# archinetai/audio-diffusion-pytorch

Hardware: AMD Instinct MI355X
Metric: denoising steps/s (UNetV0 fwd+bwd) at [B,2,2**18] (higher is better)
Workload: dtype f32; 1 GPU; BASELINE.json configs[1]: unconditional DiffusionModel(UNetV0 channels=[8,32,64,128,256,512,512,1024,1024], factors=[1,4,4,4,2,2,2,2,2], items=[1,2,2,2,2,2,2,4,4]) fwd+bwd, audio=randn(4,2,2**18) per GPU, random-init weights; per_gpu_batch=4, global_batch=4, length=262144, launch=hipGraph replay, parallelism=single, collective_world_size=1, collectives_in_graph=False, optimizer=none (the metric is fwd+bwd; gradients for all 176M parameters are produced)

## Files before the change

audio_diffusion_pytorch_amd/csrc/norm.hip:

```cpp
#include <stdlib.h>
#include "adp_rt.h"
#include "adp.h"

namespace {

constexpr int GN_CHUNK = 4096;

__global__ __launch_bounds__(256) void gn_partial_kernel(const float* x, int64_t NG, int64_t nchunks, float* ws) {
  __shared__ float sh[4];
  const int64_t bg = blockIdx.y, c = blockIdx.x;
  const float* base = x + bg * NG + c * GN_CHUNK;
  const int64_t cnt = (NG - c * GN_CHUNK) < GN_CHUNK ? (NG - c * GN_CHUNK) : GN_CHUNK;
  float v[16];
  float s = 0.0f;
#pragma unroll
  for (int j = 0; j < 16; ++j) {
    const int64_t i = (int64_t)j * 256 + threadIdx.x;
    v[j] = (i < cnt) ? base[i] : 0.0f;
    s += v[j];
  }
  const float mean = adp_block_sum<4>(s, sh) / (float)cnt;
  float q = 0.0f;
#pragma unroll
  for (int j = 0; j < 16; ++j) {
// ... 870 lines not shown
    f32x4 o;
#pragma unroll
    for (int k = 0; k < 4; ++k) o[k] = rstd[k] * (g[i][k] - m1[k] - xh[i][k] * m2[k]);
    if (dres) {
      const f32x4 r = *reinterpret_cast<const f32x4*>(dres + boff + (int64_t)c * L);
#pragma unroll
      for (int k = 0; k < 4; ++k) o[k] += r[k];
    }
    *reinterpret_cast<f32x4*>(dx + boff + (int64_t)c * L) = o;
  }
}

template <int LPR, int NT, int VPT>
__global__ __launch_bounds__(NT) void chan_lnv_bwd_chain_kernel(const float* x, const float* ss, int64_t bstride,
                                                                const float* stats1, const float* dxn, const float* gamma,
                                                                const float* stats2, const float* dres, int C, int L,
                                                                int NTL, float* dx, float* ws1, float* ws2) {
  constexpr int TL = 4 * LPR, RPP = NT / LPR, NW = NT / 64;
  __shared__ float red[4][NW][TL];
  const int tid = threadIdx.x, lane = tid & 63, wave = tid >> 6;
  const int lr = tid % LPR, rg = tid / LPR;
  const int tile = blockIdx.x, l0 = tile * TL + 4 * lr, b = blockIdx.y;
  const bool valid = l0 < L;
  const int64_t boff = (int64_t)b * C * L + l0;
  float mean1[4] = {0.0f, 0.0f, 0.0f, 0.0f}, rstd1[4] = {0.0f, 0.0f, 0.0f, 0.0f};
  float mean2[4] = {0.0f, 0.0f, 0.0f, 0.0f}, rstd2[4] = {0.0f, 0.0f, 0.0f, 0.0f};
  if (valid) {
    const float* sp = stats1 + ((int64_t)b * L + l0) * 2;
    const f32x4 a = *reinterpret_cast<const f32x4*>(sp), c4 = *reinterpret_cast<const f32x4*>(sp + 4);
    mean1[0] = a[0], rstd1[0] = a[1], mean1[1] = a[2], rstd1[1] = a[3];
    mean1[2] = c4[0], rstd1[2] = c4[1], mean1[3] = c4[2], rstd1[3] = c4[3];
    const float* sq = stats2 + ((int64_t)b * L + l0) * 2;
    const f32x4 e = *reinterpret_cast<const f32x4*>(sq), f4 = *reinterpret_cast<const f32x4*>(sq + 4);
    mean2[0] = e[0], rstd2[0] = e[1], mean2[1] = e[2], rstd2[1] = e[3];
    mean2[2] = f4[0], rstd2[2] = f4[1], mean2[3] = f4[2], rstd2[3] = f4[3];
  }
  const float* sb = ss + b * bstride;
  f32x4 xh[VPT], g[VPT];
  float mulv[VPT], addv[VPT];
  float s1[4] = {0.0f, 0.0f, 0.0f, 0.0f}, s2[4] = {0.0f, 0.0f, 0.0f, 0.0f};
  auto xhat2 = [&](int i, int k) {
    return (fmaf(xh[i][k], mulv[i], addv[i]) - mean2[k]) * rstd2[k];
  };
#pragma unroll
  for (int i = 0; i < VPT; ++i) {
    const int c = rg + i * RPP;
    const bool ok = valid && c < C;
    f32x4 d;
    if (ok) {
      d = *reinterpret_cast<const f32x4*>(dxn + boff + (int64_t)c * L);
      xh[i] = *reinterpret_cast<const f32x4*>(x + boff + (int64_t)c * L);
    } else {
#pragma unroll
      for (int k = 0; k < 4; ++k) d[k] = xh[i][k] = 0.0f;
    }
    mulv[i] = (c < C) ? 1.0f + sb[c] : 0.0f;
    addv[i] = (c < C) ? sb[C + c] : 0.0f;
    const float gm = (c < C) ? gamma[c] : 0.0f;
    float pa = 0.0f, pb = 0.0f;
#pragma unroll
    for (int k = 0; k < 4; ++k) {
      xh[i][k] = ok ? (xh[i][k] - mean1[k]) * rstd1[k] : 0.0f;
      const float x2 = ok ? xhat2(i, k) : 0.0f;
      g[i][k] = d[k] * gm;
      s1[k] += g[i][k];
      s2[k] = fmaf(g[i][k], x2, s2[k]);
      pa = fmaf(d[k], x2, pa);
      pb += d[k];
    }
#pragma unroll
    for (int o = 1; o < LPR; o <<= 1) {
      pa += __shfl_xor(pa, o, 64);
      pb += __shfl_xor(pb, o, 64);
    }
    if (lr == 0 && c < C) {
      ws2[(((int64_t)b * 2 + 0) * NTL + tile) * C + c] = pa;
      ws2[(((int64_t)b * 2 + 1) * NTL + tile) * C + c] = pb;
    }
  }
  auto over_channels = [&](float (&a)[4], float (&c2)[4], int stage) {
#pragma unroll
    for (int o = LPR; o < 64; o <<= 1)
#pragma unroll
      for (int k = 0; k < 4; ++k) {
        a[k] += __shfl_xor(a[k], o, 64);
        c2[k] += __shfl_xor(c2[k], o, 64);
      }
    if (NW > 1) {
      if (lane < LPR)
#pragma unroll
        for (int k = 0; k < 4; ++k) {
          red[2 * stage][wave][4 * lr + k] = a[k];
          red[2 * stage + 1][wave][4 * lr + k] = c2[k];
        }
      __syncthreads();
#pragma unroll
      for (int k = 0; k < 4; ++k) {
        float u = 0.0f, w2 = 0.0f;
#pragma unroll
        for (int w = 0; w < NW; ++w) {
          u += red[2 * stage][w][4 * lr + k];
          w2 += red[2 * stage + 1][w][4 * lr + k];
        }
        a[k] = u, c2[k] = w2;
      }
    }
#pragma unroll
    for (int k = 0; k < 4; ++k) {
      a[k] /= (float)C;
      c2[k] /= (float)C;
    }
  };
  over_channels(s1, s2, 0);
  float t1[4] = {0.0f, 0.0f, 0.0f, 0.0f}, t2[4] = {0.0f, 0.0f, 0.0f, 0.0f};
#pragma unroll
  for (int i = 0; i < VPT; ++i) {
    const int c = rg + i * RPP;
    const bool ok = valid && c < C;
    f32x4 r = f32x4{0.0f, 0.0f, 0.0f, 0.0f};
    if (ok && dres) r = *reinterpret_cast<const f32x4*>(dres + boff + (int64_t)c * L);
    float pa = 0.0f, pb = 0.0f;
#pragma unroll
    for (int k = 0; k < 4; ++k) {
      const float o = ok ? rstd2[k] * (g[i][k] - s1[k] - xhat2(i, k) * s2[k]) + r[k] : 0.0f;
      pa = fmaf(o, xh[i][k], pa);
      pb += o;
      g[i][k] = o * mulv[i];
      t1[k] += g[i][k];
      t2[k] = fmaf(g[i][k], xh[i][k], t2[k]);
    }
#pragma unroll
    for (int o = 1; o < LPR; o <<= 1) {
      pa += __shfl_xor(pa, o, 64);
      pb += __shfl_xor(pb, o, 64);
    }
    if (lr == 0 && c < C) {
      ws1[(((int64_t)b * 2 + 0) * NTL + tile) * C + c] = pa;
      ws1[(((int64_t)b * 2 + 1) * NTL + tile) * C + c] = pb;
    }
  }
  over_channels(t1, t2, 1);
  if (!valid) return;
#pragma unroll
  for (int i = 0; i < VPT; ++i) {
    const int c = rg + i * RPP;
    if (c >= C) continue;
    f32x4 o;
#pragma unroll
    for (int k = 0; k < 4; ++k) o[k] = rstd1[k] * (g[i][k] - t1[k] - xh[i][k] * t2[k]);
    *reinterpret_cast<f32x4*>(dx + boff + (int64_t)c * L) = o;
  }
}

struct LnvCfg {
  int lpr, nt, vpt;
};
static LnvCfg lnv_cfg(int64_t C, int64_t B, int64_t L, bool bwd = false) {
  if (C <= 8) return {64, 256, 2};
  if (C <= 32) return {32, 256, 4};
  if (C <= 64) return {16, 256, 4};
  if (C <= 128) return {8, 256, 4};
  if (C <= 256) {
    if (adp_knob(bwd ? "ADP_LNV_NT_BWD" : "ADP_LNV_NT", 512) == 1024) return {8, 1024, 2};
    return {8, 512, 4};
  }
  int lpr = 4;
  while (lpr > 1 && B * adp_cdiv(L, 4 * lpr) < 32) lpr >>= 1;
  if (adp_knob(bwd ? "ADP_LNV_NT_BWD" : "ADP_LNV_NT", 512) != 1024) {
    const int lp = (C <= 512 && lpr == 1) ? 2 : lpr;
    return {lp, 512, C <= 512 ? lp : 2 * lp};
  }
  if (C <= 512) return {lpr == 1 ? 2 : lpr, 1024, lpr == 4 ? 2 : 1};
  return {lpr, 1024, lpr};
}
static bool lnv_ok(int64_t L, const void* a, const void* b, const void* c, const void* d, const void* e) {
  return (L & 3) == 0 && ((reinterpret_cast<uintptr_t>(a) | reinterpret_cast<uintptr_t>(b) | reinterpret_cast<uintptr_t>(c) |
                           reinterpret_cast<uintptr_t>(d) | reinterpret_cast<uintptr_t>(e)) & 15) == 0;
}

struct LnCfg {
  int tl, nt;
};
LnCfg ln_cfg(int64_t C, int64_t B, int64_t L) {
  if (C <= 64) return {64, 256};
  if (C <= 128) return {32, 256};
  if (C <= 256) return {32, 1024};
  if (B * adp_cdiv(L, 16) >= 192) return {16, 1024};
  if (B * adp_cdiv(L, 8) >= 192) return {8, 1024};
  return {4, 1024};
}
constexpr int64_t LN_CMAX = 1024;

int launch_ln_fwd(const float* x, const float* ss, int64_t bstride, int64_t B, int64_t C, int64_t L, float eps, float* y,
                  float* stats, void* stream, const float* gam = nullptr, const float* bet = nullptr,
                  const float* gam2 = nullptr, const float* bet2 = nullptr, float* y2 = nullptr, float eps2 = 0.0f,
                  float* cy = nullptr, float* cstats = nullptr) {
  if (cy && !(lnv_ok(L, x, y, y2, stats, cy) && lnv_ok(L, cstats, nullptr, nullptr, nullptr, nullptr))) {
    const int rc = launch_ln_fwd(x, ss, bstride, B, C, L, eps, y, stats, stream);
    if (rc != ADP_OK) return rc;
    return launch_ln_fwd(y, nullptr, 0, B, C, L, eps2, cy, cstats, stream, gam, bet, gam2, bet2, y2);
  }
  if (lnv_ok(L, x, y, y2, stats, nullptr)) {
    const LnvCfg v = lnv_cfg(C, B, L);
    dim3 vgrid((unsigned)adp_cdiv(L, 4 * v.lpr), (unsigned)B);
#define ADP_LNV_FWD(LPR, NT, VPT)                                                                                     \
  if (v.lpr == LPR && v.nt == NT && v.vpt == VPT) {                                                                   \
    ADP_LAUNCH((chan_lnv_fwd_kernel<LPR, NT, VPT>), vgrid, dim3(NT), stream, x, ss, bstride, (int)C, (int)L, eps, y, \
               stats, gam, bet, gam2, bet2, y2, eps2, cy, cstats);                                                    \
    return ADP_LAUNCH_OK();                                                                                           \
  }
    ADP_LNV_FWD(64, 256, 2) ADP_LNV_FWD(32, 256, 4) ADP_LNV_FWD(16, 256, 4) ADP_LNV_FWD(8, 256, 4) ADP_LNV_FWD(8, 1024, 2)
    ADP_LNV_FWD(4, 1024, 2) ADP_LNV_FWD(2, 1024, 1) ADP_LNV_FWD(4, 1024, 4) ADP_LNV_FWD(2, 1024, 2) ADP_LNV_FWD(1, 1024, 1)
    ADP_LNV_FWD(4, 512, 4) ADP_LNV_FWD(4, 512, 8) ADP_LNV_FWD(2, 512, 2) ADP_LNV_FWD(2, 512, 4) ADP_LNV_FWD(1, 512, 2) ADP_LNV_FWD(8, 512, 4)
#undef ADP_LNV_FWD
  }
  const LnCfg k = ln_cfg(C, B, L);
  dim3 grid((unsigned)adp_cdiv(L, k.tl), (unsigned)B);
  if (k.tl == 8)
    ADP_LAUNCH((chan_ln_fwd_kernel<8, 1024, 8>), grid, dim3(1024), stream, x, ss, bstride, (int)C, (int)L, eps, y, stats, gam, bet, gam2, bet2, y2);
  else if (k.tl == 4)
    ADP_LAUNCH((chan_ln_fwd_kernel<4, 1024, 4>), grid, dim3(1024), stream, x, ss, bstride, (int)C, (int)L, eps, y, stats, gam, bet, gam2, bet2, y2);
  else if (k.tl == 64 && C <= 8)
    ADP_LAUNCH((chan_ln_fwd_kernel<64, 256, 2>), grid, dim3(256), stream, x, ss, bstride, (int)C, (int)L, eps, y, stats, gam, bet, gam2, bet2, y2);
  else if (k.tl == 64 && C <= 32)
    ADP_LAUNCH((chan_ln_fwd_kernel<64, 256, 8>), grid, dim3(256), stream, x, ss, bstride, (int)C, (int)L, eps, y, stats, gam, bet, gam2, bet2, y2);
  else if (k.tl == 64)
    ADP_LAUNCH((chan_ln_fwd_kernel<64, 256, 16>), grid, dim3(256), stream, x, ss, bstride, (int)C, (int)L, eps, y, stats, gam, bet, gam2, bet2, y2);
  else if (k.tl == 32 && k.nt == 256)
    ADP_LAUNCH((chan_ln_fwd_kernel<32, 256, 16>), grid, dim3(256), stream, x, ss, bstride, (int)C, (int)L, eps, y, stats, gam, bet, gam2, bet2, y2);
  else if (k.tl == 32)
    ADP_LAUNCH((chan_ln_fwd_kernel<32, 1024, 8>), grid, dim3(1024), stream, x, ss, bstride, (int)C, (int)L, eps, y, stats, gam, bet, gam2, bet2, y2);
  else
    ADP_LAUNCH((chan_ln_fwd_kernel<16, 1024, 16>), grid, dim3(1024), stream, x, ss, bstride, (int)C, (int)L, eps, y, stats, gam, bet, gam2, bet2, y2);
  return ADP_LAUNCH_OK();
}

int launch_ln_bwd(const float* x, const float* dy, const float* ss, int64_t bstride, const float* gamma,
                  const float* stats, const float* dres, int64_t B, int64_t C, int64_t L, float* dx, float* ws,
                  void* stream) {
  if (lnv_ok(L, x, dy, dres, dx, stats)) {
    const LnvCfg v = lnv_cfg(C, B, L, true);
    const int VNTL = (int)adp_cdiv(L, 4 * v.lpr);
    dim3 vgrid((unsigned)VNTL, (unsigned)B);
#define ADP_LNV_BWD(LPR, NT, VPT)                                                                                      \
  if (v.lpr == LPR && v.nt == NT && v.vpt == VPT) {                                                                    \
    ADP_LAUNCH((chan_lnv_bwd_kernel<LPR, NT, VPT>), vgrid, dim3(NT), stream, x, dy, ss, bstride, gamma, stats, dres,  \
               (int)C, (int)L, VNTL, dx, ws);                                                                          \
    return VNTL;                                                                                                       \
  }
    ADP_LNV_BWD(64, 256, 2) ADP_LNV_BWD(32, 256, 4) ADP_LNV_BWD(16, 256, 4) ADP_LNV_BWD(8, 256, 4) ADP_LNV_BWD(8, 1024, 2)
    ADP_LNV_BWD(4, 1024, 2) ADP_LNV_BWD(2, 1024, 1) ADP_LNV_BWD(4, 1024, 4) ADP_LNV_BWD(2, 1024, 2) ADP_LNV_BWD(1, 1024, 1)
    ADP_LNV_BWD(4, 512, 4) ADP_LNV_BWD(4, 512, 8) ADP_LNV_BWD(2, 512, 2) ADP_LNV_BWD(2, 512, 4) ADP_LNV_BWD(1, 512, 2) ADP_LNV_BWD(8, 512, 4)
#undef ADP_LNV_BWD
  }
  const LnCfg k = ln_cfg(C, B, L);
  const int NTL = (int)adp_cdiv(L, k.tl);
  dim3 grid((unsigned)NTL, (unsigned)B);
  if (k.tl == 8)
    ADP_LAUNCH((chan_ln_bwd_kernel<8, 1024, 8>), grid, dim3(1024), stream, x, dy, ss, bstride, gamma, stats, dres,
               (int)C, (int)L, NTL, dx, ws);
  else if (k.tl == 4)
    ADP_LAUNCH((chan_ln_bwd_kernel<4, 1024, 4>), grid, dim3(1024), stream, x, dy, ss, bstride, gamma, stats, dres,
               (int)C, (int)L, NTL, dx, ws);
  else if (k.tl == 64 && C <= 8)
    ADP_LAUNCH((chan_ln_bwd_kernel<64, 256, 2>), grid, dim3(256), stream, x, dy, ss, bstride, gamma, stats, dres,
               (int)C, (int)L, NTL, dx, ws);
  else if (k.tl == 64 && C <= 32)
    ADP_LAUNCH((chan_ln_bwd_kernel<64, 256, 8>), grid, dim3(256), stream, x, dy, ss, bstride, gamma, stats, dres,
               (int)C, (int)L, NTL, dx, ws);
  else if (k.tl == 64)
    ADP_LAUNCH((chan_ln_bwd_kernel<64, 256, 16>), grid, dim3(256), stream, x, dy, ss, bstride, gamma, stats, dres,
               (int)C, (int)L, NTL, dx, ws);
  else if (k.tl == 32 && k.nt == 256)
    ADP_LAUNCH((chan_ln_bwd_kernel<32, 256, 16>), grid, dim3(256), stream, x, dy, ss, bstride, gamma, stats, dres,
               (int)C, (int)L, NTL, dx, ws);
  else if (k.tl == 32)
    ADP_LAUNCH((chan_ln_bwd_kernel<32, 1024, 8>), grid, dim3(1024), stream, x, dy, ss, bstride, gamma, stats, dres,
               (int)C, (int)L, NTL, dx, ws);
  else
    ADP_LAUNCH((chan_ln_bwd_kernel<16, 1024, 16>), grid, dim3(1024), stream, x, dy, ss, bstride, gamma, stats, dres,
               (int)C, (int)L, NTL, dx, ws);
  return NTL;
}

__global__ __launch_bounds__(256) void reduce_rows_kernel(const float* ws, int64_t B, int64_t W, int64_t NT,
                                                          int64_t bstride, int sum_over_b, int accumulate,
                                                          float* out) {
  const int lane = threadIdx.x & 63, wave = threadIdx.x >> 6;
  const int64_t row = (int64_t)blockIdx.x * 4 + wave;
  const int64_t rows = sum_over_b ? W : B * W;
  if (row >= rows) return;
  float s = 0.0f;
  if (sum_over_b) {
    for (int64_t b = 0; b < B; ++b)
      for (int64_t t = lane; t < NT; t += 64) s += ws[(b * W + row) * NT + t];
  } else {
    for (int64_t t = lane; t < NT; t += 64) s += ws[row * NT + t];
  }
  s = adp_wave_sum(s);
  if (lane == 0) {
    const int64_t o = sum_over_b ? row : (row / W) * bstride + (row % W);
    out[o] = accumulate ? out[o] + s : s;
  }
}

__global__ __launch_bounds__(1024) void reduce_tiles_kernel(const float* ws, int64_t B, int64_t C, int64_t NT,
                                                            int64_t bstride, int sum_over_b, int accumulate,
                                                            float* out) {
  __shared__ float part[16][64];
  const int lane = threadIdx.x & 63, tg = threadIdx.x >> 6;
  const int64_t W = 2 * C;
  const int64_t j = (int64_t)blockIdx.x * 64 + lane;
  const int64_t bb = blockIdx.y;
  float s = 0.0f;
  if (j < W) {
    const int64_t which = j / C, c = j % C;
    const int64_t b0 = sum_over_b ? 0 : bb, b1 = sum_over_b ? B : bb + 1;
    for (int64_t b = b0; b < b1; ++b) {
      const float* p = ws + ((b * 2 + which) * NT) * C + c;
      for (int64_t t = tg; t < NT; t += 16) s += p[t * C];
    }
  }
  part[tg][lane] = s;
  __syncthreads();
  if (tg == 0 && j < W) {
    float v = 0.0f;
#pragma unroll
    for (int k = 0; k < 16; ++k) v += part[k][lane];
    const int64_t o = sum_over_b ? j : bb * bstride + j;
    out[o] = accumulate ? out[o] + v : v;
  }
}

__global__ __launch_bounds__(256) void reduce_tiles_wave_kernel(const float* ws, int64_t B, int64_t C, int64_t NT,
                                                                int64_t bstride, int sum_over_b, int accumulate,
                                                                float* out) {
  const int lane = threadIdx.x & 63, wave = threadIdx.x >> 6;
  const int64_t i = (int64_t)blockIdx.x * 4 + wave;
  const int64_t W = 2 * C;
  const int64_t total = sum_over_b ? W : B * W;
  if (i >= total) return;
  const int64_t j = i % W, which = j / C, c = j % C;
  float s = 0.0f;
  const int64_t b0 = sum_over_b ? 0 : i / W, b1 = sum_over_b ? B : b0 + 1;
  for (int64_t b = b0; b < b1; ++b) {
    const float* p = ws + ((b * 2 + which) * NT) * C + c;
    for (int64_t t = lane; t < NT; t += 64) s += p[t * C];
  }
  s = adp_wave_sum(s);
  if (lane == 0) {
    const int64_t o = sum_over_b ? j : b0 * bstride + j;
    out[o] = accumulate ? out[o] + s : s;
  }
}

static void launch_reduce_tiles(const float* ws, int64_t B, int64_t C, int64_t NT, int64_t bstride, int sum_over_b,
                                int accumulate, float* out, void* stream) {
  const int64_t total = sum_over_b ? 2 * C : B * 2 * C;
  if (NT >= 128 && C <= 64)
    ADP_LAUNCH(reduce_tiles_wave_kernel, dim3((unsigned)adp_cdiv(total, 4)), dim3(256), stream, ws, B, C, NT, bstride,
               sum_over_b, accumulate, out);
  else
    ADP_LAUNCH(reduce_tiles_kernel, dim3((unsigned)adp_cdiv(2 * C, 64), (unsigned)(sum_over_b ? 1 : B)), dim3(1024),
               stream, ws, B, C, NT, bstride, sum_over_b, accumulate, out);
}

constexpr int MOD_BATCH = 8;
struct adp_mod_batch {
  const float* ws[MOD_BATCH];
  float* out[MOD_BATCH];
};

__global__ __launch_bounds__(1024) void reduce_tiles_batch_kernel(adp_mod_batch q, int64_t C, int64_t NT, int64_t bstride) {
  __shared__ float part[16][64];
  const int lane = threadIdx.x & 63, tg = threadIdx.x >> 6;
  const int64_t W = 2 * C;
  const int64_t j = (int64_t)blockIdx.x * 64 + lane;
  const int64_t b = blockIdx.y;
  const float* ws = q.ws[blockIdx.z];
  float s = 0.0f;
  if (j < W) {
    const int64_t which = j / C, c = j % C;
    const float* p = ws + ((b * 2 + which) * NT) * C + c;
    for (int64_t t = tg; t < NT; t += 16) s += p[t * C];
  }
  part[tg][lane] = s;
  __syncthreads();
  if (tg == 0 && j < W) {
    float v = 0.0f;
#pragma unroll
    for (int k = 0; k < 16; ++k) v += part[k][lane];
    q.out[blockIdx.z][b * bstride + j] = v;
// ... 86 lines not shown
  if (B <= 0 || C <= 0 || L <= 0 || G <= 0 || C % G) return ADP_ERR_SHAPE;
  const int64_t NG = (C / G) * L, nchunks = adp_cdiv(NG, GN_CHUNK);
  if (B * G > 65535 || B * C > 65535) return ADP_ERR_SHAPE;
  ADP_LAUNCH(gn_partial_kernel, dim3((unsigned)nchunks, (unsigned)(B * G)), dim3(256), stream, x, NG, nchunks, ws);
  if ((L & 3) == 0 && ((reinterpret_cast<uintptr_t>(x) | reinterpret_cast<uintptr_t>(act)) & 15) == 0)
    return launch_gn_act_slab<2>(x, ws, gamma, beta, B, C, L, G, nchunks, eps, stats, act, stream);
  ADP_LAUNCH(gn_apply_kernel, dim3((unsigned)adp_cdiv(L, 1024), (unsigned)(B * C)), dim3(256), stream, x,
             (const float*)ws, gamma, beta, C, L, G, nchunks, eps, stats, act);
  return ADP_LAUNCH_OK();
}

extern "C" int64_t adp_row_nsplit(int64_t rows, int64_t L) { return row_nsplit(rows, L); }

extern "C" int adp_gn_silu_bwd_reduce(const float* x, const float* dact, const float* stats, const float* gamma,
                                      const float* beta, int64_t B, int64_t C, int64_t L, int64_t G, int64_t NS,
                                      float* ab, void* stream) {
  if (!x || !dact || !stats || !gamma || !beta || !ab) return ADP_ERR_NULL;
  if (B <= 0 || C <= 0 || L <= 0 || G <= 0 || C % G || NS < 1 || NS > 65535 || B * C > 65535) return ADP_ERR_SHAPE;
  int64_t CL = adp_cdiv(L, NS);
  if ((L & 3) == 0) CL = (CL + 3) & ~(int64_t)3;
  if (gn_bwd_vec_ok(x, dact, nullptr, nullptr, L, CL) && (reinterpret_cast<uintptr_t>(ab) & 7) == 0) {
    const int64_t nseg = B * C * NS;
    const int tpr = gn_bwd_tpr(CL);
    const dim3 grid((unsigned)adp_cdiv(nseg, 256 / tpr));
#define ADP_GN_RED(T) \
  ADP_LAUNCH((gn_bwd_reduce_vec_kernel<T>), grid, dim3(256), stream, x, dact, stats, gamma, beta, C, L, G, NS, CL, nseg, ab)
    if (tpr == 16) ADP_GN_RED(16);
    else if (tpr == 32) ADP_GN_RED(32);
    else if (tpr == 64) ADP_GN_RED(64);
    else ADP_GN_RED(256);
#undef ADP_GN_RED
    return ADP_LAUNCH_OK();
  }
  ADP_LAUNCH(gn_bwd_reduce_kernel, dim3((unsigned)NS, (unsigned)(B * C)), dim3(256), stream, x, dact, stats, gamma,
             beta, C, L, G, NS, CL, ab);
  return ADP_LAUNCH_OK();
}

extern "C" int adp_gn_silu_bwd_apply_ab(const float* x, const float* dact, const float* stats, const float* gamma,
                                        const float* beta, const float* ab, const float* dres, int64_t B, int64_t C,
                                        int64_t L, int64_t G, int64_t NS, int64_t NSab, float* dx, float* dgamma,
                                        float* dbeta, int64_t accumulate, void* stream) {
  if (!x || !dact || !stats || !gamma || !beta || !ab || !dx || (!dgamma != !dbeta)) return ADP_ERR_NULL;
  if (B <= 0 || C <= 0 || L <= 0 || G <= 0 || C % G || NS < 1 || NS > 65535 || NSab < 1 || B * C > 65535) return ADP_ERR_SHAPE;
  int64_t CL = adp_cdiv(L, NS);
  if ((L & 3) == 0) CL = (CL + 3) & ~(int64_t)3;
  if (gn_bwd_vec_ok(x, dact, dres, dx, L, CL) && (reinterpret_cast<uintptr_t>(ab) & 7) == 0) {
    const int64_t nseg = B * C * NS;
    const int tpr = gn_bwd_tpr(CL);
    const dim3 grid((unsigned)adp_cdiv(nseg, 256 / tpr));
#define ADP_GN_APP(T)                                                                                                  \
  ADP_LAUNCH((gn_bwd_apply_vec_kernel<T>), grid, dim3(256), stream, x, dact, stats, gamma, beta, ab, dres, C, L, G, NS, \
             CL, nseg, dx, B, dgamma, dbeta, (int)accumulate, NSab)
    if (tpr == 16) ADP_GN_APP(16);
    else if (tpr == 32) ADP_GN_APP(32);
    else if (tpr == 64) ADP_GN_APP(64);
    else ADP_GN_APP(256);
#undef ADP_GN_APP
    return ADP_LAUNCH_OK();
  }
  ADP_LAUNCH(gn_bwd_apply_kernel, dim3((unsigned)NS, (unsigned)(B * C)), dim3(256), stream, x, dact, stats, gamma,
             beta, ab, dres, C, L, G, NS, CL, dx, B, dgamma, dbeta, (int)accumulate, NSab);
  return ADP_LAUNCH_OK();
}

extern "C" int adp_gn_silu_bwd_apply(const float* x, const float* dact, const float* stats, const float* gamma,
                                     const float* beta, const float* ab, const float* dres, int64_t B, int64_t C,
                                     int64_t L, int64_t G, int64_t NS, float* dx, float* dgamma, float* dbeta,
                                     int64_t accumulate, void* stream) {
  return adp_gn_silu_bwd_apply_ab(x, dact, stats, gamma, beta, ab, dres, B, C, L, G, NS, NS, dx, dgamma, dbeta, accumulate,
                                  stream);
}

extern "C" int adp_gn_param_grad(const float* ab, int64_t B, int64_t C, int64_t NS, float* dgamma, float* dbeta,
                                 int64_t accumulate, void* stream) {
  if (!ab || !dgamma || !dbeta) return ADP_ERR_NULL;
  if (B <= 0 || C <= 0 || NS < 1) return ADP_ERR_SHAPE;
  ADP_LAUNCH(gn_param_grad_kernel, dim3((unsigned)adp_cdiv(C, 256)), dim3(256), stream, ab, B, C, NS, dgamma, dbeta,
             (int)accumulate);
  return ADP_LAUNCH_OK();
}

extern "C" int adp_modulation_fwd(const float* x, const float* ss, int64_t ss_bstride, int64_t B, int64_t C,
                                  int64_t L, float eps, float* y, float* stats, void* stream) {
  if (!x || !ss || !y || !stats) return ADP_ERR_NULL;
  if (B <= 0 || C <= 0 || L <= 0 || B > 65535 || L >= (int64_t)1 << 31) return ADP_ERR_SHAPE;
  if (C > LN_CMAX) return ADP_ERR_UNSUPPORTED;
  return launch_ln_fwd(x, ss, ss_bstride, B, C, L, eps, y, stats, stream);
}

extern "C" int adp_modulation_ln_fwd(const float* x, const float* ss, int64_t ss_bstride, int64_t B, int64_t C, int64_t L,
                                     float eps, float* y, float* stats, float eps_ln, const float* gamma, const float* beta,
                                     float* xn, const float* gamma2, const float* beta2, float* xn2, float* ln_stats,
                                     void* stream) {
  if (!x || !ss || !y || !stats || !gamma || !beta || !xn || !ln_stats) return ADP_ERR_NULL;
  if (xn2 && (!gamma2 || !beta2)) return ADP_ERR_NULL;
  if (B <= 0 || C <= 0 || L <= 0 || B > 65535 || L >= (int64_t)1 << 31) return ADP_ERR_SHAPE;
  if (C > LN_CMAX) return ADP_ERR_UNSUPPORTED;
  return launch_ln_fwd(x, ss, ss_bstride, B, C, L, eps, y, stats, stream, gamma, beta, gamma2, beta2, xn2, eps_ln, xn,
                       ln_stats);
}

extern "C" int adp_gn_finalize(const float* part, int64_t B, int64_t C, int64_t E, int64_t G, float eps, float* stats,
                               void* stream) {
  if (!part || !stats) return ADP_ERR_NULL;
  if (B <= 0 || C <= 0 || E <= 0 || G <= 0 || C % G || (C / G) % 4) return ADP_ERR_SHAPE;
  ADP_LAUNCH(gn_finalize_kernel, dim3((unsigned)(B * G)), dim3(64), stream, part, C, E, G, eps, stats);
  return ADP_LAUNCH_OK();
}

extern "C" int adp_gn_finalize_act(const float* x, const float* part, int64_t B, int64_t C, int64_t L, int64_t E,
                                   int64_t G, float eps, const float* gamma, const float* beta, float* stats,
                                   float* act, void* stream) {
  if (!x || !part || !gamma || !beta || !stats || !act) return ADP_ERR_NULL;
  if (B <= 0 || C <= 0 || L <= 0 || E <= 0 || G <= 0 || C % G || (C / G) % 4 || B * C > 65535) return ADP_ERR_SHAPE;
  if ((L & 3) == 0 && ((reinterpret_cast<uintptr_t>(x) | reinterpret_cast<uintptr_t>(act)) & 15) == 0)
    return launch_gn_act_slab<1>(x, part, gamma, beta, B, C, L, G, E, eps, stats, act, stream);
  ADP_LAUNCH(gn_finalize_act_kernel, dim3((unsigned)adp_cdiv(L, 1024), (unsigned)(B * C)), dim3(256), stream, x, part,
             gamma, beta, C, L, G, E, eps, stats, act);
  return ADP_LAUNCH_OK();
}

extern "C" int adp_gn_act(const float* x, const float* stats, const float* gamma, const float* beta, int64_t B,
                          int64_t C, int64_t L, int64_t G, float* act, void* stream) {
  if (!x || !stats || !gamma || !beta || !act) return ADP_ERR_NULL;
  if (B <= 0 || C <= 0 || L <= 0 || G <= 0 || C % G || B * C > 65535) return ADP_ERR_SHAPE;
  if ((L & 3) == 0 && ((reinterpret_cast<uintptr_t>(x) | reinterpret_cast<uintptr_t>(act)) & 15) == 0)
    return launch_gn_act_slab<0>(x, stats, gamma, beta, B, C, L, G, 0, 0.0f, (float*)nullptr, act, stream);
  ADP_LAUNCH(gn_act_kernel, dim3((unsigned)adp_cdiv(L, 1024), (unsigned)(B * C)), dim3(256), stream, x, stats, gamma,
             beta, C, L, G, act);
  return ADP_LAUNCH_OK();
}

extern "C" int adp_ln_stats(const float* x, int64_t B, int64_t C, int64_t L, float eps, float* stats, void* stream) {
  if (!x || !stats) return ADP_ERR_NULL;
  if (B <= 0 || C <= 0 || L <= 0 || B > 65535 || L >= (int64_t)1 << 31) return ADP_ERR_SHAPE;
  if (C > LN_CMAX) return ADP_ERR_UNSUPPORTED;
  return launch_ln_fwd(x, (const float*)nullptr, (int64_t)0, B, C, L, eps, (float*)nullptr, stats, stream);
}

extern "C" int adp_ln_affine_fwd(const float* x, int64_t B, int64_t C, int64_t L, float eps, const float* gamma,
                                 const float* beta, float* y, const float* gamma2, const float* beta2, float* y2,
                                 float* stats, void* stream) {
  if (!x || !gamma || !beta || !y || !stats) return ADP_ERR_NULL;
  if (y2 && (!gamma2 || !beta2)) return ADP_ERR_NULL;
  if (B <= 0 || C <= 0 || L <= 0 || B > 65535 || L >= (int64_t)1 << 31) return ADP_ERR_SHAPE;
  if (C > LN_CMAX) return ADP_ERR_UNSUPPORTED;
  return launch_ln_fwd(x, (const float*)nullptr, (int64_t)0, B, C, L, eps, y, stats, stream, gamma, beta, gamma2, beta2,
                       y2);
}

extern "C" int64_t adp_chan_ln_bwd_ws_bytes(int64_t B, int64_t C, int64_t L) {
  if (B <= 0 || C <= 0 || L <= 0) return ADP_ERR_SHAPE;
  const int64_t t_old = adp_cdiv(L, ln_cfg(C, B, L).tl), t_vec = adp_cdiv(L, 4 * lnv_cfg(C, B, L).lpr);
  return B * 2 * C * (t_old > t_vec ? t_old : t_vec) * (int64_t)sizeof(float);
}

extern "C" int adp_modulation_bwd(const float* x, const float* dy, const float* ss, int64_t ss_bstride,
                                  const float* stats, int64_t B, int64_t C, int64_t L, float* dx, float* dss,
                                  int64_t dss_bstride, float* ws, void* stream) {
  if (!x || !dy || !ss || !stats || !dx || !dss || !ws) return ADP_ERR_NULL;
  if (B <= 0 || C <= 0 || L <= 0 || B > 65535 || L >= (int64_t)1 << 31) return ADP_ERR_SHAPE;
  if (C > LN_CMAX) return ADP_ERR_UNSUPPORTED;
  const int64_t NT = launch_ln_bwd(x, dy, ss, ss_bstride, (const float*)nullptr, stats, (const float*)nullptr, B, C, L, dx,
                                   ws, stream);
  launch_reduce_tiles((const float*)ws, B, C, NT, dss_bstride, 0, 0, dss, stream);
  return ADP_LAUNCH_OK();
}

extern "C" int64_t adp_modulation_bwd_partial(const float* x, const float* dy, const float* ss, int64_t ss_bstride,
                                              const float* stats, int64_t B, int64_t C, int64_t L, float* dx, float* ws,
                                              void* stream) {
  if (!x || !dy || !ss || !stats || !dx || !ws) return ADP_ERR_NULL;
  if (B <= 0 || C <= 0 || L <= 0 || B > 65535 || L >= (int64_t)1 << 31) return ADP_ERR_SHAPE;
  if (C > LN_CMAX) return ADP_ERR_UNSUPPORTED;
  const int64_t NT = launch_ln_bwd(x, dy, ss, ss_bstride, (const float*)nullptr, stats, (const float*)nullptr, B, C, L, dx,
                                   ws, stream);
  return ADP_LAUNCH_OK() == ADP_OK ? NT : (int64_t)ADP_ERR_LAUNCH;
}

extern "C" int adp_modulation_bwd_reduce(const float* const* ws, float* const* dss, int64_t n, int64_t B, int64_t C,
                                         int64_t NT, int64_t dss_bstride, void* stream) {
  if (!ws || !dss) return ADP_ERR_NULL;
  if (n < 1 || B <= 0 || C <= 0 || NT <= 0 || B > 65535) return ADP_ERR_SHAPE;
  for (int64_t at = 0; at < n; at += MOD_BATCH) {
    adp_mod_batch q;
    const int m = (int)(n - at < MOD_BATCH ? n - at : MOD_BATCH);
    for (int i = 0; i < MOD_BATCH; ++i) {
      q.ws[i] = ws[at + (i < m ? i : 0)];
      q.out[i] = dss[at + (i < m ? i : 0)];
      if (!q.ws[i] || !q.out[i]) return ADP_ERR_NULL;
    }
    if (NT >= 128 && C <= 64)
      ADP_LAUNCH(reduce_tiles_wave_batch_kernel, dim3((unsigned)adp_cdiv(B * 2 * C, 4), 1, (unsigned)m), dim3(256), stream, q,
                 B, C, NT, dss_bstride);
    else
      ADP_LAUNCH(reduce_tiles_batch_kernel, dim3((unsigned)adp_cdiv(2 * C, 64), (unsigned)B, (unsigned)m), dim3(1024),
                 stream, q, C, NT, dss_bstride);
  }
  return ADP_LAUNCH_OK();
}

extern "C" int adp_ln_bwd(const float* x, const float* dxn, const float* stats, const float* gamma, const float* dres,
                          int64_t B, int64_t C, int64_t L, int64_t accumulate, float* dx, float* dgamma_dbeta,
                          float* ws, void* stream) {
  if (!x || !dxn || !stats || !gamma || !dx || !dgamma_dbeta || !ws) return ADP_ERR_NULL;
  if (B <= 0 || C <= 0 || L <= 0 || B > 65535 || L >= (int64_t)1 << 31) return ADP_ERR_SHAPE;
  if (C > LN_CMAX) return ADP_ERR_UNSUPPORTED;
  const int64_t NT = launch_ln_bwd(x, dxn, (const float*)nullptr, (int64_t)0, gamma, stats, dres, B, C, L, dx, ws, stream);
  launch_reduce_tiles((const float*)ws, B, C, NT, (int64_t)0, 1, (int)accumulate, dgamma_dbeta, stream);
  return ADP_LAUNCH_OK();
}

extern "C" int64_t adp_modulation_ln_bwd_partial(const float* x, const float* ss, int64_t ss_bstride, const float* stats,
                                                 const float* y, const float* dxn, const float* gamma, const float* ln_stats,
                                                 const float* dres, int64_t B, int64_t C, int64_t L, int64_t accumulate,
                                                 float* dx, float* ws, float* dgamma_dbeta, float* ws_ln, void* stream) {
  if (!x || !ss || !stats || !y || !dxn || !gamma || !ln_stats || !dx || !ws || !dgamma_dbeta || !ws_ln) return ADP_ERR_NULL;
  if (B <= 0 || C <= 0 || L <= 0 || B > 65535 || L >= (int64_t)1 << 31) return ADP_ERR_SHAPE;
  if (C > LN_CMAX) return ADP_ERR_UNSUPPORTED;
  int64_t NT = -1;
  if (lnv_ok(L, x, dxn, dres, dx, stats) && lnv_ok(L, ln_stats, nullptr, nullptr, nullptr, nullptr)) {
    const LnvCfg v = lnv_cfg(C, B, L, true);
    const int VNTL = (int)adp_cdiv(L, 4 * v.lpr);
    dim3 vgrid((unsigned)VNTL, (unsigned)B);
#define ADP_LNV_CHAIN(LPR, NT_, VPT)                                                                                    \
  if (NT < 0 && v.lpr == LPR && v.nt == NT_ && v.vpt == VPT) {                                                          \
    ADP_LAUNCH((chan_lnv_bwd_chain_kernel<LPR, NT_, VPT>), vgrid, dim3(NT_), stream, x, ss, ss_bstride, stats, dxn,    \
               gamma, ln_stats, dres, (int)C, (int)L, VNTL, dx, ws, ws_ln);                                             \
    NT = VNTL;                                                                                                          \
  }
    ADP_LNV_CHAIN(64, 256, 2) ADP_LNV_CHAIN(32, 256, 4) ADP_LNV_CHAIN(16, 256, 4) ADP_LNV_CHAIN(8, 256, 4) ADP_LNV_CHAIN(8, 1024, 2)
    ADP_LNV_CHAIN(4, 1024, 2) ADP_LNV_CHAIN(2, 1024, 1) ADP_LNV_CHAIN(4, 1024, 4) ADP_LNV_CHAIN(2, 1024, 2) ADP_LNV_CHAIN(1, 1024, 1)
    ADP_LNV_CHAIN(4, 512, 4) ADP_LNV_CHAIN(4, 512, 8) ADP_LNV_CHAIN(2, 512, 2) ADP_LNV_CHAIN(2, 512, 4) ADP_LNV_CHAIN(1, 512, 2) ADP_LNV_CHAIN(8, 512, 4)
#undef ADP_LNV_CHAIN
    if (NT > 0) launch_reduce_tiles((const float*)ws_ln, B, C, NT, (int64_t)0, 1, (int)accumulate, dgamma_dbeta, stream);
  }
  if (NT < 0) {
    const int64_t NA = launch_ln_bwd(y, dxn, (const float*)nullptr, (int64_t)0, gamma, ln_stats, dres, B, C, L, dx, ws_ln, stream);
    launch_reduce_tiles((const float*)ws_ln, B, C, NA, (int64_t)0, 1, (int)accumulate, dgamma_dbeta, stream);
    NT = launch_ln_bwd(x, dx, ss, ss_bstride, (const float*)nullptr, stats, (const float*)nullptr, B, C, L, dx, ws, stream);
  }
  return ADP_LAUNCH_OK() == ADP_OK ? NT : (int64_t)ADP_ERR_LAUNCH;
}

extern "C" int64_t adp_skipmod_bwd_ws_bytes(int64_t B, int64_t C, int64_t L) {
  if (B <= 0 || C <= 0 || L <= 0) return ADP_ERR_SHAPE;
  return B * C * row_nsplit(B * C, L) * (int64_t)sizeof(float);
}

extern "C" int adp_skipmod_bwd(const float* g, const float* x, const float* scale, int64_t scale_bstride, int64_t B,
                               int64_t C, int64_t L, float* dx, float* dscale, int64_t dscale_bstride, float* ws,
                               void* stream) {
  if (!g || !x || !scale || !dx || !dscale || !ws) return ADP_ERR_NULL;
  if (B <= 0 || C <= 0 || L <= 0 || B * C > 65535) return ADP_ERR_SHAPE;
  const int64_t NS = row_nsplit(B * C, L), CL = adp_cdiv(L, NS);
  ADP_LAUNCH(skipmod_bwd_kernel, dim3((unsigned)NS, (unsigned)(B * C)), dim3(256), stream, g, x, scale,
             scale_bstride, C, L, NS, CL, dx, ws);
  ADP_LAUNCH(reduce_rows_kernel, dim3((unsigned)adp_cdiv(B * C, 4)), dim3(256), stream, (const float*)ws, B, C, NS,
             dscale_bstride, 0, 0, dscale);
  return ADP_LAUNCH_OK();
}
```

Measured before the change: 91.27 denoising steps/s.

## Split channel LayerNorm across channel groups for low-occupancy deep layers

Adds a channel-split path for channel LayerNorm forward and backward when C is 512-1024 and there are few length tiles. Each call becomes two kernels over a 3D grid with a channel-split dimension. The first writes partial sums, using a pivoted shifted-variance scheme in forward, into scratch space (the output buffer in forward, extra workspace in backward). The second combines the partials Chan-style and applies the normalization. This spreads work across more CUs for the small-L, wide-channel levels, at the cost of an extra launch and re-reading the input.

```diff
diff --git a/audio_diffusion_pytorch_amd/csrc/norm.hip b/audio_diffusion_pytorch_amd/csrc/norm.hip
--- a/audio_diffusion_pytorch_amd/csrc/norm.hip
+++ b/audio_diffusion_pytorch_amd/csrc/norm.hip
@@ -1046,6 +1046,308 @@
   }
 }
 
+struct LnsCfg {
+  int vpt, cs;
+};
+static LnsCfg lns_cfg(int64_t C, int64_t B, int64_t L) {
+  const int64_t tiles = B * adp_cdiv(L, 16);
+  if (C < 512 || C > 1024 || tiles < 32 || tiles >= 192) return {0, 0};
+  for (int vpt = 2; vpt <= 4; vpt += 2) {
+    if (vpt == 2 && C > 512 && tiles * adp_cdiv(C, 256) >= 192) continue;
+    const int64_t cw = 64 * vpt, cs = adp_cdiv(C, cw);
+    if (C - (cs - 1) * cw >= 2 * cs) return {vpt, (int)cs};
+  }
+  return {0, 0};
+}
+constexpr int LNS_MAXCS = 8;
+
+__device__ __forceinline__ void lns_over_channels(float (&t)[4], float (*red)[16], int lane, int wave, int lr) {
+#pragma unroll
+  for (int o = 4; o < 64; o <<= 1)
+#pragma unroll
+    for (int k = 0; k < 4; ++k) t[k] += __shfl_xor(t[k], o, 64);
+  if (lane < 4)
+#pragma unroll
+    for (int k = 0; k < 4; ++k) red[wave][4 * lr + k] = t[k];
+  __syncthreads();
+#pragma unroll
+  for (int k = 0; k < 4; ++k) t[k] = (red[0][4 * lr + k] + red[1][4 * lr + k]) + (red[2][4 * lr + k] + red[3][4 * lr + k]);
+}
+
+__device__ __forceinline__ f32x4 lns_pivot(f32x4 v) {
+#pragma unroll
+  for (int k = 0; k < 4; ++k) v[k] = rintf(v[k] * 0.015625f) * 64.0f;
+  return v;
+}
+
+template <int VPT>
+__global__ __launch_bounds__(256) void chan_lns_fwd_part_kernel(const float* x, int C, int L, float* y) {
+  constexpr int CW = 64 * VPT;
+  __shared__ float red2[2][4][16];
+  const int tid = threadIdx.x, lane = tid & 63, wave = tid >> 6, lr = tid & 3, rg = tid >> 2;
+  const int l0 = blockIdx.x * 16 + 4 * lr, b = blockIdx.y, split = blockIdx.z, c0 = split * CW, CS = gridDim.z;
+  const bool valid = l0 < L;
+  const int nc = C - c0 < CW ? C - c0 : CW;
+  const float* xb = x + (int64_t)b * C * L + l0;
+  f32x4 x0 = f32x4{0.0f, 0.0f, 0.0f, 0.0f};
+  if (valid) x0 = lns_pivot(*reinterpret_cast<const f32x4*>(xb));
+  f32x4 v[VPT];
+  float s[4] = {0.0f, 0.0f, 0.0f, 0.0f};
+#pragma unroll
+  for (int i = 0; i < VPT; ++i) {
+    const int c = c0 + rg + i * 64;
+    if (valid && c < C) {
+      v[i] = *reinterpret_cast<const f32x4*>(xb + (int64_t)c * L);
+    } else {
+      v[i] = x0;
+    }
+#pragma unroll
+    for (int k = 0; k < 4; ++k) {
+      v[i][k] -= x0[k];
+      s[k] += v[i][k];
+    }
+  }
+  lns_over_channels(s, red2[0], lane, wave, lr);
+  float q[4] = {0.0f, 0.0f, 0.0f, 0.0f};
+#pragma unroll
+  for (int i = 0; i < VPT; ++i) {
+    const bool in = c0 + rg + i * 64 < C;
+#pragma unroll
+    for (int k = 0; k < 4; ++k) {
+      const float dlt = in ? v[i][k] - s[k] / (float)nc : 0.0f;
+      q[k] = fmaf(dlt, dlt, q[k]);
+    }
+  }
+  lns_over_channels(q, red2[1], lane, wave, lr);
+  if (tid < 4 * CS && valid) {
+    float* p = y + ((int64_t)b * C + (tid >> 2) * CW + 2 * split) * L + l0;
+    *reinterpret_cast<f32x4*>(p) = f32x4{s[0], s[1], s[2], s[3]};
+    *reinterpret_cast<f32x4*>(p + L) = f32x4{q[0], q[1], q[2], q[3]};
+  }
+}
+
+template <int VPT>
+__global__ __launch_bounds__(256) void chan_lns_fwd_apply_kernel(const float* x, const float* ss, int64_t bstride, int C,
+                                                                 int L, float eps, float* y, float* stats, const float* gam,
+                                                                 const float* bet, const float* gam2, const float* bet2,
+                                                                 float* y2) {
+  constexpr int CW = 64 * VPT;
+  __shared__ float mr[2][16];
+  const int tid = threadIdx.x, lr = tid & 3, rg = tid >> 2;
+  const int l0 = blockIdx.x * 16 + 4 * lr, b = blockIdx.y, c0 = blockIdx.z * CW, CS = gridDim.z;
+  const bool valid = l0 < L;
+  const bool aff = gam != nullptr;
+  const float* xb = x + (int64_t)b * C * L + l0;
+  const float* sb = ss ? ss + b * bstride : nullptr;
+  f32x4 v[VPT];
+  float mulv[VPT], addv[VPT];
+#pragma unroll
+  for (int i = 0; i < VPT; ++i) {
+    const int c = c0 + rg + i * 64;
+    mulv[i] = addv[i] = 0.0f;
+    if (c < C) {
+      mulv[i] = aff ? gam[c] : 1.0f + sb[c];
+      addv[i] = aff ? bet[c] : sb[C + c];
+    }
+    if (valid && c < C) {
+      v[i] = *reinterpret_cast<const f32x4*>(xb + (int64_t)c * L);
+    } else {
+#pragma unroll
+      for (int k = 0; k < 4; ++k) v[i][k] = 0.0f;
+    }
+  }
+  if (tid < 4) {
+    float mean[4] = {0.0f, 0.0f, 0.0f, 0.0f}, rstd[4] = {0.0f, 0.0f, 0.0f, 0.0f};
+    if (valid) {
+      const float* p = y + ((int64_t)b * C + c0) * L + l0;
+      const f32x4 x0 = lns_pivot(*reinterpret_cast<const f32x4*>(xb));
+      f32x4 ps[LNS_MAXCS], pm[LNS_MAXCS];
+#pragma unroll
+      for (int sp = 0; sp < LNS_MAXCS; ++sp)
+        if (sp < CS) {
+          ps[sp] = *reinterpret_cast<const f32x4*>(p + (int64_t)(2 * sp) * L);
+          pm[sp] = *reinterpret_cast<const f32x4*>(p + (int64_t)(2 * sp + 1) * L);
+        }
+      float n = 0.0f, S[4] = {0.0f, 0.0f, 0.0f, 0.0f}, M[4] = {0.0f, 0.0f, 0.0f, 0.0f};
+#pragma unroll
+      for (int sp = 0; sp < LNS_MAXCS; ++sp)
+        if (sp < CS) {
+          const float nb = (float)(C - sp * CW < CW ? C - sp * CW : CW);
+#pragma unroll
+          for (int k = 0; k < 4; ++k) {
+            if (sp == 0) {
+              S[k] = ps[sp][k], M[k] = pm[sp][k];
+            } else {
+              const float dlt = ps[sp][k] / nb - S[k] / n;
+              M[k] += pm[sp][k] + dlt * dlt * (n * nb / (n + nb));
+              S[k] += ps[sp][k];
+            }
+          }
+          n += nb;
+        }
+#pragma unroll
+      for (int k = 0; k < 4; ++k) {
+        mean[k] = x0[k] + S[k] / (float)C;
+        rstd[k] = 1.0f / sqrtf(M[k] / (float)C + eps);
+      }
+      if (blockIdx.z == 0) {
+        float* sp = stats + ((int64_t)b * L + l0) * 2;
+        *reinterpret_cast<f32x4*>(sp) = f32x4{mean[0], rstd[0], mean[1], rstd[1]};
+        *reinterpret_cast<f32x4*>(sp + 4) = f32x4{mean[2], rstd[2], mean[3], rstd[3]};
+      }
+    }
+#pragma unroll
+    for (int k = 0; k < 4; ++k) mr[0][4 * tid + k] = mean[k], mr[1][4 * tid + k] = rstd[k];
+  }
+  __syncthreads();
+  if (!valid) return;
+  float mean[4], rstd[4];
+#pragma unroll
+  for (int k = 0; k < 4; ++k) mean[k] = mr[0][4 * lr + k], rstd[k] = mr[1][4 * lr + k];
+  float* yb = y + (int64_t)b * C * L + l0;
+  float* yb2 = y2 ? y2 + (int64_t)b * C * L + l0 : nullptr;
+#pragma unroll
+  for (int i = 0; i < VPT; ++i) {
+    const int c = c0 + rg + i * 64;
+    if (c >= C) continue;
+    f32x4 o;
+#pragma unroll
+    for (int k = 0; k < 4; ++k) o[k] = fmaf((v[i][k] - mean[k]) * rstd[k], mulv[i], addv[i]);
+    *reinterpret_cast<f32x4*>(yb + (int64_t)c * L) = o;
+    if (yb2) {
+      const float m2 = gam2[c], a2 = bet2[c];
+#pragma unroll
+      for (int k = 0; k < 4; ++k) o[k] = fmaf((v[i][k] - mean[k]) * rstd[k], m2, a2);
+      *reinterpret_cast<f32x4*>(yb2 + (int64_t)c * L) = o;
+    }
+  }
+}
+
+template <int VPT>
+__global__ __launch_bounds__(256) void chan_lns_bwd_part_kernel(const float* x, const float* dy, const float* ss,
+                                                                int64_t bstride, const float* gamma, const float* stats,
+                                                                int C, int L, int NTL, float* ws, float* part) {
+  constexpr int CW = 64 * VPT;
+  __shared__ float red[2][4][16];
+  const int tid = threadIdx.x, lane = tid & 63, wave = tid >> 6, lr = tid & 3, rg = tid >> 2;
+  const int tile = blockIdx.x, l0 = tile * 16 + 4 * lr, b = blockIdx.y, split = blockIdx.z, c0 = split * CW;
+  const bool valid = l0 < L;
+  const int64_t boff = (int64_t)b * C * L + l0;
+  float mean[4] = {0.0f, 0.0f, 0.0f, 0.0f}, rstd[4] = {0.0f, 0.0f, 0.0f, 0.0f};
+  if (valid) {
+    const float* sp = stats + ((int64_t)b * L + l0) * 2;
+    const f32x4 a = *reinterpret_cast<const f32x4*>(sp), c4 = *reinterpret_cast<const f32x4*>(sp + 4);
+    mean[0] = a[0], rstd[0] = a[1], mean[1] = a[2], rstd[1] = a[3];
+    mean[2] = c4[0], rstd[2] = c4[1], mean[3] = c4[2], rstd[3] = c4[3];
+  }
+  f32x4 d[VPT], xv[VPT];
+  float mul[VPT];
+#pragma unroll
+  for (int i = 0; i < VPT; ++i) {
+    const int c = c0 + rg + i * 64;
+    if (valid && c < C) {
+      d[i] = *reinterpret_cast<const f32x4*>(dy + boff + (int64_t)c * L);
+      xv[i] = *reinterpret_cast<const f32x4*>(x + boff + (int64_t)c * L);
+    } else {
+#pragma unroll
+      for (int k = 0; k < 4; ++k) d[i][k] = xv[i][k] = 0.0f;
+    }
+    mul[i] = (c < C) ? (gamma ? gamma[c] : 1.0f + ss[b * bstride + c]) : 0.0f;
+  }
+  float s1[4] = {0.0f, 0.0f, 0.0f, 0.0f}, s2[4] = {0.0f, 0.0f, 0.0f, 0.0f};
+#pragma unroll
+  for (int i = 0; i < VPT; ++i) {
+    const int c = c0 + rg + i * 64;
+    const bool ok = valid && c < C;
+    float pa = 0.0f, pb = 0.0f;
+#pragma unroll
+    for (int k = 0; k < 4; ++k) {
+      const float xh = ok ? (xv[i][k] - mean[k]) * rstd[k] : 0.0f;
+      const float g = d[i][k] * mul[i];
+      s1[k] += g;
+      s2[k] = fmaf(g, xh, s2[k]);
+      pa = fmaf(d[i][k], xh, pa);
+      pb += d[i][k];
+    }
+#pragma unroll
+    for (int o = 1; o < 4; o <<= 1) {
+      pa += __shfl_xor(pa, o, 64);
+      pb += __shfl_xor(pb, o, 64);
+    }
+    if (lr == 0 && c < C) {
+      ws[(((int64_t)b * 2 + 0) * NTL + tile) * C + c] = pa;
+      ws[(((int64_t)b * 2 + 1) * NTL + tile) * C + c] = pb;
+    }
+  }
+  lns_over_channels(s1, red[0], lane, wave, lr);
+  lns_over_channels(s2, red[1], lane, wave, lr);
+  if (tid < 4) {
+    float* p = part + ((((int64_t)b * NTL + tile) * gridDim.z + split) * 2) * 16 + 4 * tid;
+    *reinterpret_cast<f32x4*>(p) = f32x4{s1[0], s1[1], s1[2], s1[3]};
+    *reinterpret_cast<f32x4*>(p + 16) = f32x4{s2[0], s2[1], s2[2], s2[3]};
+  }
+}
+
+template <int VPT>
+__global__ __launch_bounds__(256) void chan_lns_bwd_apply_kernel(const float* x, const float* dy, const float* ss,
+                                                                 int64_t bstride, const float* gamma, const float* stats,
+                                                                 const float* dres, int C, int L, int NTL, float* dx,
+                                                                 const float* part) {
+  constexpr int CW = 64 * VPT;
+  const int tid = threadIdx.x, lr = tid & 3, rg = tid >> 2;
+  const int tile = blockIdx.x, l0 = tile * 16 + 4 * lr, b = blockIdx.y, c0 = blockIdx.z * CW, CS = gridDim.z;
+  if (l0 >= L) return;
+  const int64_t boff = (int64_t)b * C * L + l0;
+  const float* sp = stats + ((int64_t)b * L + l0) * 2;
+  const f32x4 a = *reinterpret_cast<const f32x4*>(sp), c4 = *reinterpret_cast<const f32x4*>(sp + 4);
+  const float mean[4] = {a[0], a[2], c4[0], c4[2]}, rstd[4] = {a[1], a[3], c4[1], c4[3]};
+  f32x4 d[VPT], xv[VPT], r[VPT];
+  float mul[VPT];
+#pragma unroll
+  for (int i = 0; i < VPT; ++i) {
+    const int c = c0 + rg + i * 64;
+#pragma unroll
+    for (int k = 0; k < 4; ++k) d[i][k] = xv[i][k] = r[i][k] = 0.0f;
+    mul[i] = 0.0f;
+    if (c < C) {
+      d[i] = *reinterpret_cast<const f32x4*>(dy + boff + (int64_t)c * L);
+      xv[i] = *reinterpret_cast<const f32x4*>(x + boff + (int64_t)c * L);
+      if (dres) r[i] = *reinterpret_cast<const f32x4*>(dres + boff + (int64_t)c * L);
+      mul[i] = gamma ? gamma[c] : 1.0f + ss[b * bstride + c];
+    }
+  }
+  float m1[4] = {0.0f, 0.0f, 0.0f, 0.0f}, m2[4] = {0.0f, 0.0f, 0.0f, 0.0f};
+  {
+    const float* p = part + (((int64_t)b * NTL + tile) * CS * 2) * 16 + 4 * lr;
+    f32x4 p1[LNS_MAXCS], p2[LNS_MAXCS];
+#pragma unroll
+    for (int s = 0; s < LNS_MAXCS; ++s)
+      if (s < CS) {
+        p1[s] = *reinterpret_cast<const f32x4*>(p + s * 32);
+        p2[s] = *reinterpret_cast<const f32x4*>(p + s * 32 + 16);
+      }
+#pragma unroll
+    for (int s = 0; s < LNS_MAXCS; ++s)
+      if (s < CS)
+#pragma unroll
+        for (int k = 0; k < 4; ++k) m1[k] += p1[s][k], m2[k] += p2[s][k];
+#pragma unroll
+    for (int k = 0; k < 4; ++k) m1[k] /= (float)C, m2[k] /= (float)C;
+  }
+#pragma unroll
+  for (int i = 0; i < VPT; ++i) {
+    const int c = c0 + rg + i * 64;
+    if (c >= C) continue;
+    f32x4 o;
+#pragma unroll
+    for (int k = 0; k < 4; ++k) {
+      const float xh = (xv[i][k] - mean[k]) * rstd[k];
+      o[k] = rstd[k] * (d[i][k] * mul[i] - m1[k] - xh * m2[k]) + r[i][k];
+    }
+    *reinterpret_cast<f32x4*>(dx + boff + (int64_t)c * L) = o;
+  }
+}
+
 struct LnvCfg {
   int lpr, nt, vpt;
 };
@@ -1084,6 +1386,10 @@
   return {4, 1024};
 }
 constexpr int64_t LN_CMAX = 1024;
+static int64_t ln_bwd_ws_tiles(int64_t B, int64_t C, int64_t L) {
+  const int64_t t_old = adp_cdiv(L, ln_cfg(C, B, L).tl), t_vec = adp_cdiv(L, 4 * lnv_cfg(C, B, L).lpr);
+  return t_old > t_vec ? t_old : t_vec;
+}
 
 int launch_ln_fwd(const float* x, const float* ss, int64_t bstride, int64_t B, int64_t C, int64_t L, float eps, float* y,
                   float* stats, void* stream, const float* gam = nullptr, const float* bet = nullptr,
@@ -1093,6 +1399,23 @@
     const int rc = launch_ln_fwd(x, ss, bstride, B, C, L, eps, y, stats, stream);
     if (rc != ADP_OK) return rc;
     return launch_ln_fwd(y, nullptr, 0, B, C, L, eps2, cy, cstats, stream, gam, bet, gam2, bet2, y2);
+  }
+  if (!cy && y && lnv_ok(L, x, y, y2, stats, nullptr)) {
+    const LnsCfg sc = lns_cfg(C, B, L);
+    const float* ye = y + B * C * L;
+    if (sc.cs && (x + B * C * L <= y || ye <= x)) {
+      dim3 sgrid((unsigned)adp_cdiv(L, 16), (unsigned)B, (unsigned)sc.cs);
+      if (sc.vpt == 2) {
+        ADP_LAUNCH((chan_lns_fwd_part_kernel<2>), sgrid, dim3(256), stream, x, (int)C, (int)L, y);
+        ADP_LAUNCH((chan_lns_fwd_apply_kernel<2>), sgrid, dim3(256), stream, x, ss, bstride, (int)C, (int)L, eps, y, stats,
+                   gam, bet, gam2, bet2, y2);
+      } else {
+        ADP_LAUNCH((chan_lns_fwd_part_kernel<4>), sgrid, dim3(256), stream, x, (int)C, (int)L, y);
+        ADP_LAUNCH((chan_lns_fwd_apply_kernel<4>), sgrid, dim3(256), stream, x, ss, bstride, (int)C, (int)L, eps, y, stats,
+                   gam, bet, gam2, bet2, y2);
+      }
+      return ADP_LAUNCH_OK();
+    }
   }
   if (lnv_ok(L, x, y, y2, stats, nullptr)) {
     const LnvCfg v = lnv_cfg(C, B, L);
@@ -1132,6 +1455,26 @@
 int launch_ln_bwd(const float* x, const float* dy, const float* ss, int64_t bstride, const float* gamma,
                   const float* stats, const float* dres, int64_t B, int64_t C, int64_t L, float* dx, float* ws,
                   void* stream) {
+  if (lnv_ok(L, x, dy, dres, dx, stats) && (reinterpret_cast<uintptr_t>(ws) & 15) == 0) {
+    const LnsCfg sc = lns_cfg(C, B, L);
+    if (sc.cs) {
+      const int SNTL = (int)adp_cdiv(L, 16);
+      float* part = ws + B * 2 * C * ln_bwd_ws_tiles(B, C, L);
+      dim3 sgrid((unsigned)SNTL, (unsigned)B, (unsigned)sc.cs);
+      if (sc.vpt == 2) {
+        ADP_LAUNCH((chan_lns_bwd_part_kernel<2>), sgrid, dim3(256), stream, x, dy, ss, bstride, gamma, stats, (int)C, (int)L,
+                   SNTL, ws, part);
+        ADP_LAUNCH((chan_lns_bwd_apply_kernel<2>), sgrid, dim3(256), stream, x, dy, ss, bstride, gamma, stats, dres, (int)C,
+                   (int)L, SNTL, dx, (const float*)part);
+      } else {
+        ADP_LAUNCH((chan_lns_bwd_part_kernel<4>), sgrid, dim3(256), stream, x, dy, ss, bstride, gamma, stats, (int)C, (int)L,
+                   SNTL, ws, part);
+        ADP_LAUNCH((chan_lns_bwd_apply_kernel<4>), sgrid, dim3(256), stream, x, dy, ss, bstride, gamma, stats, dres, (int)C,
+                   (int)L, SNTL, dx, (const float*)part);
+      }
+      return SNTL;
+    }
+  }
   if (lnv_ok(L, x, dy, dres, dx, stats)) {
     const LnvCfg v = lnv_cfg(C, B, L, true);
     const int VNTL = (int)adp_cdiv(L, 4 * v.lpr);
@@ -1524,8 +1867,8 @@
 
 extern "C" int64_t adp_chan_ln_bwd_ws_bytes(int64_t B, int64_t C, int64_t L) {
   if (B <= 0 || C <= 0 || L <= 0) return ADP_ERR_SHAPE;
-  const int64_t t_old = adp_cdiv(L, ln_cfg(C, B, L).tl), t_vec = adp_cdiv(L, 4 * lnv_cfg(C, B, L).lpr);
-  return B * 2 * C * (t_old > t_vec ? t_old : t_vec) * (int64_t)sizeof(float);
+  const int64_t pairs = B * adp_cdiv(L, 16) * lns_cfg(C, B, L).cs * 32;
+  return (B * 2 * C * ln_bwd_ws_tiles(B, C, L) + pairs) * (int64_t)sizeof(float);
 }
 
 extern "C" int adp_modulation_bwd(const float* x, const float* dy, const float* ss, int64_t ss_bstride,
```

Measured after the change: 89.64 denoising steps/s. -1.8%, worse.
